# fperezgamonal/flownet2-tf

Hardware: AMD Instinct MI355X
Metric: forward pairs/sec at 512x384 (FlowNet2) (higher is better)
Workload: dtype f16x2 (split fp16 hi+lo operands, 3 fp16 MFMAs per product, fp32 accumulate); 1 GPU; FlowNet2 forward, batch=4 synthetic 512x384 pairs per GPU, seeded synthetic weights; pairs_per_gpu=4, parallelism=dp1 (no collective)

## Files before the change

flownet2-tf_amd/csrc/conv.hip:

```cpp
#include "conv_common.h"
#include <cstdlib>

namespace fn2 {

template <typename T, typename OutT, int TC, int WC, int WP>
__global__ void __launch_bounds__(256) conv_igemm_kernel(const ConvArgs p) {
  constexpr int CH = 16 / (int)sizeof(T);
  constexpr int BC = WC * TC * 16;
  constexpr int BP = WP * 64;
  constexpr int NT = 256;
  static_assert(WC * WP == 4, "4 waves per block");
  constexpr int NPR = BP / 64;
  constexpr int NWR = (BC * 4 + NT - 1) / NT;
  constexpr int WSWZ_BIT = (TC == 4) ? 5 : (TC == 2) ? 4 : 3;
  __shared__ uint4 lds[2][(BC + BP) * 4];

  const int tid = threadIdx.x, lane = tid & 63, wave = tid >> 6;
  const int wc = wave / WP, wp = wave % WP;
  const int cid = tid & 3;

  int pad_y = p.pad, pad_x = p.pad, oy_off = 0, ox_off = 0, osc = 1;
  const T* wgt = reinterpret_cast<const T*>(p.wgt);
  const int phase = blockIdx.z / p.splitk, split = blockIdx.z - phase * p.splitk;
  if (p.deconv) {
// ... 808 lines not shown

}

namespace fn2 {

static bool is_flow_head(const fn2_conv_desc* d) {
  return d->kind == 0 && d->out.c == 2 && d->kh == 3 && d->kw == 3 && d->stride == 1 && d->pad == 1 &&
         d->out.dtype == FN2_F32 && d->act == FN2_ACT_NONE;
}

static bool wants_bp64(const ConvArgs& a, int tile, int phases, int layout) {
  if (layout != 1 || (a.dbg & 32)) return false;
  if (tile < 128) return true;
  const char* e = getenv("FN2_BP64_MIN");
  const int min_blocks = e ? atoi(e) : 96;
  return cdiv(a.M, 64) * (long)(a.cout_pad / 128) * phases >= min_blocks;
}

static int build_args(const fn2_conv_desc* d, ConvArgs* out, int* tile_out, int* phases_out) {
  FN2_REQUIRE(d, "conv2d: null descriptor");
  int rc = check_view(&d->in, "conv2d input");
  if (rc) return rc;
  rc = check_view(&d->out, "conv2d output");
  if (rc) return rc;
  FN2_REQUIRE(d->wgt, "conv2d: null weights");
  FN2_REQUIRE((d->kind >= 0 && d->kind <= 3) || d->kind == 5,
              "conv2d: kind must be 0 (conv), 1 (deconv k4 s2 crop 1), 2 (stem row-run conv), 3 (transpose of a stride-2 conv) "
              "or 5 (deconv k4 s2 crop 1, column phases merged)");
  FN2_REQUIRE(d->in.n == d->out.n, "conv2d: batch mismatch");
  FN2_REQUIRE(d->up_src == nullptr || ((d->kind == 1 || d->kind == 5) && d->up_w != nullptr && d->up_c0 >= 0 &&
                                       d->up_c0 + 2 <= d->out.cs && !d->accumulate),
              "conv2d: up_src rides on a kind-1 / kind-5 transposed conv (up_w set, [up_c0, up_c0 + 2) inside the out buffer)");
  FN2_REQUIRE(d->cin_pad % 8 == 0 && d->cin_pad >= d->in.c, "conv2d: cin_pad must be a multiple of 8 >= Cin");
  FN2_REQUIRE(d->in.cs % 8 == 0 && d->in.c0 % 8 == 0, "conv2d: input channel stride/offset must be multiples of 8");
  if (d->kind != 2)
    FN2_REQUIRE(d->in.c0 + d->cin_pad <= d->in.cs, "conv2d: padded input channels exceed the buffer stride");
  const int esz = dtype_size(d->in.dtype);
  const int CH = 16 / esz;
  FN2_REQUIRE(d->kpad > 0 && d->kpad % (4 * CH) == 0, "conv2d: kpad must be a multiple of one k-step");
  fn2_conv_plan plan;
  rc = fn2_conv2d_plan(d->in.dtype, d->cin_pad, d->out.c, &plan);
  if (rc) return rc;
  const bool wfrag = d->wgt_layout == 2;
  if (wfrag)
    FN2_REQUIRE(plan.layout == 1 && plan.cout_tile >= 64 && d->in.dtype == FN2_F16X2 && d->kind != 2,
                "conv2d: wgt_layout 2 (fragment order) is for split-fp16 layers with more than 32 output channels");
  else
    FN2_REQUIRE(d->wgt_layout == plan.layout, "conv2d: wgt_layout %d does not match fn2_conv2d_plan (%d)", d->wgt_layout,
                plan.layout);
  const int tile = plan.cout_tile;
  FN2_REQUIRE(d->cout_pad % tile == 0 && d->cout_pad >= d->out.c, "conv2d: cout_pad must be a multiple of the cout tile");
  FN2_REQUIRE(d->act == FN2_ACT_NONE || d->act == FN2_ACT_LEAKY, "conv2d: bad activation");
  FN2_REQUIRE(d->out.dtype == d->in.dtype || d->out.dtype == FN2_F32 ||
                  (d->in.dtype == FN2_F32 && d->out.dtype == FN2_F16X2),
              "conv2d: output dtype must be the input dtype, fp32, or split-fp16 from an fp32 stem");
  if (d->in.dtype == FN2_F16X2) FN2_REQUIRE(d->in.cs % 8 == 0 && d->in.c0 % 8 == 0, "conv2d: split-fp16 views are group (8) aligned");
  if (d->out.dtype == FN2_F16X2) FN2_REQUIRE(d->out.cs % 8 == 0 && d->out.c0 % 8 == 0, "conv2d: split-fp16 views are group (8) aligned");

  ConvArgs& a = *out;
  a = ConvArgs{};
  a.KH_KW_hint = 0;
  a.wfrag = wfrag ? 1 : 0;
  a.merged = d->kind == 5 ? 1 : 0;
  a.in = d->in.data; a.wgt = d->wgt; a.bias = d->bias; a.out = d->out.data;
  a.N = d->in.n; a.H = d->in.h; a.W = d->in.w; a.in_cs = d->in.cs; a.in_c0 = d->in.c0;
  a.cin_chunks = d->cin_pad / CH;
  int phases = 1;
  int trim[2] = {0, 0};
  if (d->kind == 0) {
    FN2_REQUIRE(d->kh >= 1 && d->kw >= 1 && d->stride >= 1 && d->pad >= 0, "conv2d: bad kernel geometry");
    a.KH = d->kh; a.KW = d->kw; a.stride = d->stride; a.pad = d->pad;
    a.OH = (d->in.h + 2 * d->pad - d->kh) / d->stride + 1;
    a.OW = (d->in.w + 2 * d->pad - d->kw) / d->stride + 1;
    FN2_REQUIRE(a.OH >= 1 && a.OW >= 1, "conv2d: kernel does not fit");
    FN2_REQUIRE(d->out.h == a.OH && d->out.w == a.OW, "conv2d: output spatial size %dx%d != expected %dx%d",
                d->out.h, d->out.w, a.OH, a.OW);
    a.deconv = 0; a.ph_pad0 = a.ph_pad1 = 0;
  } else if (d->kind == 2) {
    FN2_REQUIRE(d->kh >= 1 && d->kw >= 1 && d->stride >= 1 && d->pad == 0, "stem conv: pad must be baked into the input buffer");
    FN2_REQUIRE(d->in.c0 == 0 && d->in.c == d->in.cs, "stem conv: the input view must be the whole buffer");
    FN2_REQUIRE(d->cin_pad >= d->kw * d->in.cs, "stem conv: run (cin_pad) shorter than kw*cs");
    FN2_REQUIRE(d->wgt_layout == 1, "stem conv: runs on the LDS-DMA kernel only (run must be whole 128-byte lines)");
    a.KH = d->kh; a.KW = 1; a.stride = d->stride; a.pad = 0;
    a.KH_KW_hint = d->kw;
    a.OH = (d->in.h - d->kh) / d->stride + 1;
    a.OW = (d->in.w - d->kw) / d->stride + 1;
    FN2_REQUIRE(a.OH >= 1 && a.OW >= 1, "stem conv: kernel does not fit");
    FN2_REQUIRE(d->out.h == a.OH && d->out.w == a.OW, "stem conv: output spatial size %dx%d != expected %dx%d",
                d->out.h, d->out.w, a.OH, a.OW);
// ... 86 lines not shown
  a.kg = 1;
  if (d->wgt_layout == 1 && tile == 128 && !(a.dbg & 32)) {
    const char* e_kg = getenv("FN2_KG");
    if (!e_kg || atoi(e_kg) != 0) {
      const char* e3 = getenv("FN2_KG3_MAX");
      const char* e2 = getenv("FN2_KG2_MAX");
      const long blocks = (long)cdiv(a.M, 64) * (a.cout_pad / 128) * phases;
      if (blocks <= (e3 ? atoi(e3) : 0)) { a.bp64 = 1; a.kg = 3; }
      else if (blocks <= (e2 ? atoi(e2) : 95)) { a.bp64 = 1; a.kg = 2; }
    }
  }
  if (d->wgt_layout == 1 && tile == 128 && !(a.dbg & 32) && d->in.dtype == FN2_F16X2) {
    const char* e_lo = getenv("FN2_DEEP_MIN");
    const char* e_hi = getenv("FN2_DEEP_MAX");
    const long blocks = (long)cdiv(a.M, 64) * (a.cout_pad / 128) * phases;
    const int lo = e_lo ? atoi(e_lo) : 0, hi = e_hi ? atoi(e_hi) : -1;
    if (blocks >= lo && blocks <= hi) { a.bp64 = 3; a.kg = 1; }
  }
  if (d->wgt_layout == 1 && tile == 128 && a.bp64 == 1 && a.kg == 1) {
    const char* e_ring = getenv("FN2_RING_MAX");
    const int ring_max = e_ring ? atoi(e_ring) : 512;
    const long blocks = (long)cdiv(a.M, 64) * (a.cout_pad / 128) * phases;
    if ((a.dbg & 256) || (blocks >= 384 && blocks <= ring_max)) a.bp64 = 2;
    const char* e_rs = getenv("FN2_RING_SPLIT");
    if (e_rs && blocks >= atoi(e_rs) && blocks < 384) a.bp64 = 2;
  }
  *tile_out = tile;
  *phases_out = phases;
  return FN2_OK;
}

static int preferred_split(const ConvArgs& a, int tile, int phases) {
  if (a.merged) return 1;
  const int bp = tile == 128 ? (a.bp64 ? 64 : 128) : (a.bp64 ? 128 : 256);
  const long blocks = (long)cdiv(a.M, bp) * (a.cout_pad / tile) * phases;
  const char* e_min = getenv("FN2_SPLIT_MINBLOCKS");
  if (blocks >= (e_min ? atoi(e_min) : 384)) return 1;
  if (a.bp64 == 3) {
    const char* e_sl = getenv("FN2_DEEP_SLOTS");
    int s = (int)((e_sl ? atoi(e_sl) : 256) / blocks);
    const int maxs = a.ksteps / 16;
    if (s > maxs) s = maxs;
    if (s > 16) s = 16;
    if (s < 2) return 1;
    const int kper = cdiv(a.ksteps, s);
    return cdiv(a.ksteps, kper);
  }
  if (a.kg > 1) {
    const char* e_nos = getenv("FN2_KG_NOSPLIT");
    if (blocks >= (e_nos ? atoi(e_nos) : 96)) return 1;
    const char* e_sl = getenv("FN2_KG_SLOTS");
    int s = (int)((e_sl ? atoi(e_sl) : 256) / blocks);
    const int maxs = a.ksteps / (12 * a.kg);
    if (s > maxs) s = maxs;
    if (s > 16) s = 16;
    if (s < 2) return 1;
    const int kper = cdiv(a.ksteps, s);
    return cdiv(a.ksteps, kper);
  }
  const char* e = getenv("FN2_SPLIT_SLOTS");
  const char* e_rsl = getenv("FN2_RING_SPLIT_SLOTS");
  const int slots = (tile == 128 && a.bp64 == 2) ? (e_rsl ? atoi(e_rsl) : 512) : e ? atoi(e) : 640;
  int s = (int)(slots / blocks);
  const int maxs = a.ksteps / 8;
  if (s > maxs) s = maxs;
  if (s > 16) s = 16;
// ... 349 lines not shown
```

flownet2-tf_amd/csrc/conv2.hip:

```cpp
#include "conv_common.h"

#include <type_traits>
#include <algorithm>
#include <utility>

#ifndef FN2_X2_ORDER
#define FN2_X2_ORDER 0
#endif
#ifndef FN2_CONV_ABLATE
#define FN2_CONV_ABLATE 0
#endif
#ifndef FN2_SETPRIO
#define FN2_SETPRIO 1
#endif

namespace fn2 {

typedef __attribute__((address_space(3))) void* lptr_t;

constexpr unsigned kOobOffset = 0x80000000u;

typedef int v4i_t __attribute__((ext_vector_type(4)));
typedef unsigned u32x4_t __attribute__((ext_vector_type(4)));

// ... 1348 lines not shown
        av[k] = accr[ai[k]];
      }
#pragma unroll
      for (int k = 0; k < 2; ++k) {
        const int it = min(wave + 8 * k, 9);
        const int ky = it >> 1, o = it & 1;
        const int y = r + 2 - ky;
        float sum = tv[k][0];
        sum += tv[k][1];
        sum += tv[k][2];
        sum += tv[k][3];
        sum += tv[k][4];
        const float v = av[k] + sum;
        if (ok[k]) {
          accr[ai[k]] = fin[k] ? 0.f : v;
          const int ox = x0 + x;
          if (fin[k] && ox < W && !(p.h5_ring && (y == 0 || y == H - 1 || ox == 0 || ox == W - 1)))
            pf[(((size_t)n * H + y) * W + ox) * 2 + o] = v + bias_o[o];
        }
      }
    }
  }
  asm volatile("s_waitcnt vmcnt(0)" ::: "memory");
  if (p.h5_wc != nullptr && !(p.dbg & 16)) {
    const long total = (long)p.N * (2 * W + 2 * (H - 2));
    const long per = (total + gridDim.x - 1) / gridDim.x;
    const long m1 = min(total, (long)(b + 1) * per);
    for (long m = (long)b * per + wave; m < m1; m += 8) h5_ring_pixel(p, m);
  }
#endif
}


template <typename OutT, int SPP>
__global__ void __launch_bounds__(256) conv_rowrun_kernel(const ConvArgs p, const int npieces) {
#if defined(__HIP_DEVICE_COMPILE__)
  using T = x2_t;
  constexpr int BC = 64, BP = 128, TCN = 2;
  constexpr int MAXP = SPP == 4 ? 17 : 9;
  __shared__ uint4 ldsA[2][BC * 8];
  __shared__ uint4 ldsB[2][MAXP * 64];
  const int tid = threadIdx.x, lane = tid & 63;
  const int wave = __builtin_amdgcn_readfirstlane(tid >> 6);
  const T* wgt = reinterpret_cast<const T*>(p.wgt);
  const unsigned wrow_bytes = (unsigned)p.ksteps * 128u;
  int bx = blockIdx.x, by = blockIdx.y;
  {
    const int NT = gridDim.x * gridDim.y, L = blockIdx.x + gridDim.x * blockIdx.y;
    const int xcd = L & 7, chunk = NT >> 3, rem = NT & 7;
    const int Lp = xcd * chunk + min(xcd, rem) + (L >> 3);
    bx = Lp / (int)gridDim.y;
    by = Lp - bx * (int)gridDim.y;
  }
  const int m0 = bx * BP, c0 = by * BC;
  const int tn = m0 / (p.OH * p.OW);
  const int trem = m0 - tn * (p.OH * p.OW);
  const int toy = trem / p.OW, tox = trem - toy * p.OW;

  const v4i_t rsrc_w = make_rsrc(wgt, (int)(p.cout_pad * wrow_bytes));
  const v4i_t rsrc_x = make_rsrc(p.in, p.in_bytes);
  const int lrow = lane >> 3, lphys = lane & 7;
  unsigned woff[2];
#pragma unroll
  for (int j = 0; j < 2; ++j) {
    const int row = wave * 16 + j * 8 + lrow;
    woff[j] = (unsigned)(c0 + row) * wrow_bytes + (unsigned)((lphys ^ ((row >> 1) & 7)) * 16);
  }
  const int nslots = ((BP - 1) * p.stride + p.KH_KW_hint) * SPP;
  const int seg0 = (((tn * p.H + toy * p.stride) * p.W + tox * p.stride) * p.in_cs + p.in_c0) * 4;
  constexpr int NBW = (MAXP + 3) / 4;
  unsigned boff[NBW];
#pragma unroll
  for (int j = 0; j < NBW; ++j) {
    const int q = wave + 4 * j;
    const int P = q * 64 + lane;
    const int Ls = P ^ ((P >> 4) & 15);
    boff[j] = (q < npieces && Ls < nslots) ? (unsigned)(seg0 + Ls * 16) : kOobOffset;
  }
  const int nl = p.cin_chunks >> 3;
  const int ngroups = (p.KH_KW_hint * p.in_cs + 7) >> 3;
  auto issue_B = [&](int ky, uint4* lds) {
    const int toff = ky * p.W * p.in_cs * 4;
#pragma unroll
    for (int j = 0; j < NBW; ++j) {
      const int q = wave + 4 * j;
      if (q < npieces) dma16(rsrc_x, &lds[q * 64], boff[j] == kOobOffset ? kOobOffset : boff[j] + (unsigned)toff, 0);
    }
  };
  auto issue_A = [&](int ky, int l, uint4* lds) {
    const int soff = (ky * nl + l) * 128;
#pragma unroll
    for (int j = 0; j < 2; ++j) dma16(rsrc_w, &lds[(wave * 16 + j * 8) * 8], woff[j], soff);
  };

  const int fr = lane & 31, fh = lane >> 5, fsw = (fr >> 1) & 7;
  const int pslot = (wave * 32 + fr) * p.stride * SPP;
  f32x16 acc[TCN];
#pragma unroll
  for (int tc = 0; tc < TCN; ++tc)
#pragma unroll
    for (int q = 0; q < 16; ++q) acc[tc][q] = 0.f;

  issue_B(0, ldsB[0]);
  issue_A(0, 0, ldsA[0]);
  asm volatile("s_waitcnt vmcnt(0)" ::: "memory");
  __syncthreads();
  int abuf = 0;
  for (int ky = 0; ky < p.KH; ++ky) {
    const uint4* lb = ldsB[ky & 1];
    for (int l = 0; l < nl; ++l) {
      if (l + 1 < nl) issue_A(ky, l + 1, ldsA[abuf ^ 1]);
      else if (ky + 1 < p.KH) issue_A(ky + 1, 0, ldsA[abuf ^ 1]);
      if (l == 0 && ky + 1 < p.KH) issue_B(ky + 1, ldsB[(ky + 1) & 1]);
#if FN2_SETPRIO
      __builtin_amdgcn_s_setprio(1);
#endif
      const uint4* A = &ldsA[abuf][fr * 8];
#pragma unroll
      for (int q = 0; q < 2; ++q) {
        if (4 * l + 2 * q >= ngroups) continue;
        const int chh = (4 * q + 2 * fh) ^ fsw, chl = (4 * q + 2 * fh + 1) ^ fsw;
        const int g = 4 * l + 2 * q + fh;
        const int sh = pslot + 2 * g, sl = sh + 1;
        const uint4 bh = lb[sh ^ ((sh >> 4) & 15)], bl = lb[sl ^ ((sl >> 4) & 15)];
#pragma unroll
        for (int tc = 0; tc < TCN; ++tc) {
          const uint4 ah = A[tc * 32 * 8 + chh], al = A[tc * 32 * 8 + chl];
          acc[tc] = mfma_32x32x16<f16_t>(al, bh, acc[tc]);
          acc[tc] = mfma_32x32x16<f16_t>(ah, bl, acc[tc]);
          acc[tc] = mfma_32x32x16<f16_t>(ah, bh, acc[tc]);
        }
      }
#if FN2_SETPRIO
      __builtin_amdgcn_s_setprio(0);
#endif
      asm volatile("s_waitcnt vmcnt(0)" ::: "memory");
      __syncthreads();
      abuf ^= 1;
    }
  }

  OutT* out = reinterpret_cast<OutT*>(p.out);
  const bool vec16 = (p.out_cs % 8 == 0) && (p.out_c0 % 8 == 0);
  const int ox = tox + wave * 32 + fr;
  constexpr int ERS = 36;
  float* const tl = reinterpret_cast<float*>(&ldsB[0][0]) + wave * (32 * ERS);
  static_assert(4 * 32 * ERS * 4 <= (int)sizeof(ldsB), "epilogue tiles fit the segment buffers");
#pragma unroll
  for (int tc = 0; tc < TCN; ++tc) {
    const int cout_base = c0 + tc * 32 + fh * 16;
    OutT* po = out + (((size_t)tn * p.out_H + toy) * p.out_W + ox) * p.out_cs + p.out_c0 + cout_base;
    float v[16];
#pragma unroll
    for (int q = 0; q < 16; ++q) {
      float x = acc[tc][q] * p.out_scale + ((p.bias != nullptr && cout_base + q < p.Cout) ? p.bias[cout_base + q] : 0.f);
      if (p.act == FN2_ACT_LEAKY) x = leaky(x);
      v[q] = x;
    }
    if (sizeof(OutT) == 4 && vec16 && c0 + tc * 32 + 32 <= p.Cout && !(p.dbg & 4194304)) {
      store16<OutT>(reinterpret_cast<OutT*>(tl + fr * ERS + fh * 16), v);
      const int rr = lane >> 3, ch = lane & 7;
      OutT* ob = out + (((size_t)tn * p.out_H + toy) * p.out_W + tox + wave * 32) * p.out_cs + p.out_c0 + c0 + tc * 32 + ch * 4;
#pragma unroll
      for (int i = 0; i < 4; ++i) {
        const int row = i * 8 + rr;
        *reinterpret_cast<uint4*>(ob + (size_t)row * p.out_cs) = *reinterpret_cast<const uint4*>(tl + row * ERS + ch * 4);
      }
    } else if (vec16 && cout_base + 15 < p.Cout) {
      store16<OutT>(po, v);
    } else {
#pragma unroll
      for (int q = 0; q < 16; ++q)
        if (cout_base + q < p.Cout) store_elem<OutT>(po + q, v[q]);
    }
  }
#endif
}

template <typename OutT>
static bool launch_rowrun(const ConvArgs& a, int tile, int phases, hipStream_t s) {
  if ((a.dbg & 65536) || tile != 64 || phases != 1 || a.deconv || a.KW != 1 || a.KH_KW_hint < 1 || a.splitk != 1 || a.accum || a.wfrag)
    return false;
  if (a.OW % 128 != 0 || (a.in_cs != 8 && a.in_cs != 16)) return false;
  const int spp = a.in_cs / 4;
  const int nl = a.cin_chunks >> 3;
  const int max_slot = 127 * a.stride * spp + 2 * (4 * nl - 1) + 1;
  const int npieces = max_slot / 64 + 1;
  if (npieces > (spp == 4 ? 17 : 9)) return false;
  dim3 grid(a.M / 128, a.cout_pad / 64, 1), block(256);
  if (conv_name_sink().buf) {
    snprintf(conv_name_sink().buf, conv_name_sink().cap, "conv_rowrun_kernel<%s, %d>", is_x2<OutT>::value ? "fn2::x2_t" : "float", spp);
    return true;
  }
  if (spp == 4) hipLaunchKernelGGL((conv_rowrun_kernel<OutT, 4>), grid, block, 0, s, a, npieces);
  else hipLaunchKernelGGL((conv_rowrun_kernel<OutT, 2>), grid, block, 0, s, a, npieces);
  return true;
}

template <typename OutT>
static bool launch_stem(const ConvArgs& a, int tile, int phases, hipStream_t s) {
  if ((a.dbg & 8192) || tile != 64 || phases != 1 || a.deconv || a.KW != 1 || a.splitk != 1 || a.accum ||
      a.ksteps < 1 || a.ksteps > 4 || a.cout_pad != 64)
    return false;
  const int ntiles = cdiv(a.M, 128);
  if (ntiles < 512) return false;
  const char* e = getenv("FN2_STEM_BLOCKS");
  const int blocks = std::min(ntiles, e ? atoi(e) : 256);
  if (conv_name_sink().buf) {
    snprintf(conv_name_sink().buf, conv_name_sink().cap, "conv_stem_kernel<%s, %d>",
             is_x2<OutT>::value ? "fn2::x2_t" : "float", a.ksteps);
    return true;
  }
  switch (a.ksteps) {
    case 1: hipLaunchKernelGGL((conv_stem_kernel<OutT, 1>), dim3(blocks), dim3(256), 0, s, a, ntiles); break;
    case 2: hipLaunchKernelGGL((conv_stem_kernel<OutT, 2>), dim3(blocks), dim3(256), 0, s, a, ntiles); break;
    case 3: hipLaunchKernelGGL((conv_stem_kernel<OutT, 3>), dim3(blocks), dim3(256), 0, s, a, ntiles); break;
    default: hipLaunchKernelGGL((conv_stem_kernel<OutT, 4>), dim3(blocks), dim3(256), 0, s, a, ntiles); break;
  }
  return true;
}

template <typename OutT>
static bool launch_halo(const ConvArgs& a, int tile, int phases, hipStream_t s) {
  if (((a.dbg & 2048) && !a.merged) || a.stride != 1 || a.splitk != 1 || a.kg != 1 || !a.bp64 || a.wfrag || (a.KW != 2 && a.KW != 3)) return false;
  if (a.deconv && (a.kh_ph[0] != a.KH || a.kh_ph[1] != a.KH || a.kw_ph[0] != a.KW || a.kw_ph[1] != a.KW)) return false;
  if (tile == 128 && a.bp64 == 2 && !(a.dbg & 4096)) return false;
  if (a.bp64 == 3) return false;
// ... 114 lines not shown
  if (conv_name_sink().buf) FN2_CONV_NAME("head5_strip_kernel<%d>", a.ksteps / 3);
  else if (a.ksteps == 3) hipLaunchKernelGGL((head5_strip_kernel<1>), dim3(blocks), dim3(512), 0, s, a);
  else hipLaunchKernelGGL((head5_strip_kernel<2>), dim3(blocks), dim3(512), 0, s, a);
  return conv_launched("flow_head5_strip");
}

int launch_head5(const ConvArgs& a, int blocks, hipStream_t s) {
  if (conv_name_sink().buf)
    FN2_CONV_NAME("conv_igemm2_kernel<fn2::x2_t, float, 1, 4, 2, 2, 2, 1, false, false, false, true>");
  else
    hipLaunchKernelGGL((conv_igemm2_kernel<x2_t, float, 1, 4, 2, 2, 2, 1, false, false, false, true>), dim3(blocks, 1, 1), dim3(256), 0,
                       s, a);
  return conv_launched("flow_head5");
}

bool conv_fast_ok(int in_dtype, int cin_pad, int cout) {
  const int esz = dtype_size(in_dtype);
  return cout > 2 && (cin_pad * esz) % 128 == 0;
}

int launch_conv_fast(const ConvArgs& a, int in_dtype, int out_dtype, int tile, int phases, hipStream_t s) {
  if (tile != 128 && tile != 64 && tile != 32) return fail(FN2_ERR_UNSUPPORTED, "conv fast path: cout tile %d", tile);
  if (in_dtype == FN2_F32) return launch2<float, float>(a, tile, phases, s);
  if (in_dtype == FN2_BF16) {
    if (out_dtype == FN2_BF16) return launch2<bf16_t, bf16_t>(a, tile, phases, s);
    return launch2<bf16_t, float>(a, tile, phases, s);
  }
  if (in_dtype == FN2_F16) {
    if (out_dtype == FN2_F16) return launch2<f16_t, f16_t>(a, tile, phases, s);
    return launch2<f16_t, float>(a, tile, phases, s);
  }
  if (out_dtype == FN2_F16X2) {
    if (launch_rowrun<x2_t>(a, tile, phases, s)) return conv_launched("conv_rowrun");
    if (launch_stem<x2_t>(a, tile, phases, s)) return conv_launched("conv_stem");
    if (launch_halo<x2_t>(a, tile, phases, s)) return conv_launched("conv_halo");
    if (a.merged) return fail(FN2_ERR_UNSUPPORTED, "conv2d kind 5: needs the halo kernel (input width a multiple of 128, no split-K)");
    return launch2<x2_t, x2_t>(a, tile, phases, s);
  }
  if (launch_halo<float>(a, tile, phases, s)) return conv_launched("conv_halo");
  if (a.merged) return fail(FN2_ERR_UNSUPPORTED, "conv2d kind 5: needs the halo kernel (input width a multiple of 128, no split-K)");
  return launch2<x2_t, float>(a, tile, phases, s);
}

}
```

flownet2-tf_amd/csrc/elem.hip:

```cpp
#include "fn2_common.h"

namespace fn2 {

__device__ __forceinline__ void warp3(const float* __restrict__ img, long nb, int x, int y, float u, float v,
                                      int W, int H, float o[3]) {
  const float x2 = (float)x + u, y2 = (float)y + v;
  o[0] = o[1] = o[2] = 0.f;
  if (!((x2 >= 0.f) && (y2 >= 0.f) && (x2 < (float)W) && (y2 < (float)H))) return;
  const int xL = (int)x2, yT = (int)y2;
  const int xR = min(xL + 1, W - 1), yB = min(yT + 1, H - 1);
  const float al = x2 - (float)xL, be = y2 - (float)yT;
  const float cTL = (1.f - al) * (1.f - be), cTR = al * (1.f - be), cBL = (1.f - al) * be, cBR = al * be;
  const rgb3_t tl = load_rgb(img + (nb + (long)yT * W + xL) * 3), tr = load_rgb(img + (nb + (long)yT * W + xR) * 3);
  const rgb3_t bl = load_rgb(img + (nb + (long)yB * W + xL) * 3), br = load_rgb(img + (nb + (long)yB * W + xR) * 3);
  o[0] = cTL * tl.r + cTR * tr.r + cBL * bl.r + cBR * br.r;
  o[1] = cTL * tl.g + cTR * tr.g + cBL * bl.g + cBR * br.g;
  o[2] = cTL * tl.b + cTR * tr.b + cBL * bl.b + cBR * br.b;
}

struct FlowSrc { const float* p; int ph, pw; float sy, sx, scale; float* keep; };

__device__ __forceinline__ float2 flow_at(const FlowSrc& f, int n, int y, int x, long pix) {
  if (f.ph == 0) return *reinterpret_cast<const float2*>(f.p + pix * 2);
  const float fy = (float)y * f.sy;
  const int y0 = (int)floorf(fy);
  const int y1 = min(y0 + 1, f.ph - 1);
  const float ly = fy - (float)y0;
  const float2* r0 = reinterpret_cast<const float2*>(f.p) + ((long)n * f.ph + y0) * f.pw;
  const float2* r1 = reinterpret_cast<const float2*>(f.p) + ((long)n * f.ph + y1) * f.pw;
  const float fx = (float)x * f.sx;
  const int x0 = (int)floorf(fx);
  const int x1 = min(x0 + 1, f.pw - 1);
  const float lx = fx - (float)x0;
  float2 r = bilerp_c2(r0[x0], r0[x1], r1[x0], r1[x1], lx, ly, f.scale);
  asm volatile("" : "+v"(r.x), "+v"(r.y));
  if (f.keep != nullptr) *reinterpret_cast<float2*>(f.keep + pix * 2) = r;
  return r;
}

template <typename OutT>
__global__ void __launch_bounds__(256) stack_input_kernel(const float* __restrict__ a, const float* __restrict__ b,
                                                          const FlowSrc flow, OutT* __restrict__ out,
                                                          int N, int H, int W, int out_cs, int out_c0, int pad) {
  const long npix = (long)N * H * W;
  for (long pix = (long)blockIdx.x * blockDim.x + threadIdx.x; pix < npix; pix += (long)gridDim.x * blockDim.x) {
    const int x = (int)(pix % W), y = (int)((pix / W) % H);
    const long nb = (pix / W / H) * (long)H * W;
    const float2 f = flow_at(flow, (int)(pix / W / H), y, x, pix);
    float wv[3];
    warp3(b, nb, x, y, f.x, f.y, W, H, wv);
    float v[16];
    float e = 0.f;
    const rgb3_t pa = load_rgb(a + pix * 3), pb = load_rgb(b + pix * 3);
    const float av3[3] = {pa.r, pa.g, pa.b}, bv3[3] = {pb.r, pb.g, pb.b};
#pragma unroll
    for (int c = 0; c < 3; ++c) {
      const float av = av3[c];
      v[c] = av;
      v[3 + c] = bv3[c];
      v[6 + c] = wv[c];
      const float d = av - wv[c];
      e += d * d;
    }
    v[9] = f.x * 0.05f;
    v[10] = f.y * 0.05f;
    v[11] = sqrtf(e);
    v[12] = v[13] = v[14] = v[15] = 0.f;
    const size_t opix = ((size_t)(pix / W / H) * (H + 2 * pad) + y + pad) * (W + 2 * pad) + x + pad;
    store16<OutT>(out + opix * out_cs + out_c0, v);
  }
}

template <typename OutT>
__global__ void __launch_bounds__(256) fusion_input_kernel(const float* __restrict__ a, const float* __restrict__ b,
                                                           const FlowSrc fsd, const FlowSrc fcss, OutT* __restrict__ out,
                                                           int N, int H, int W, int out_cs, int out_c0, int pad) {
  const long npix = (long)N * H * W;
  for (long pix = (long)blockIdx.x * blockDim.x + threadIdx.x; pix < npix; pix += (long)gridDim.x * blockDim.x) {
    const int x = (int)(pix % W), y = (int)((pix / W) % H);
    const long nb = (pix / W / H) * (long)H * W;
    const float2 sd = flow_at(fsd, (int)(pix / W / H), y, x, pix);
    const float2 cs = flow_at(fcss, (int)(pix / W / H), y, x, pix);
    float wsd[3], wcs[3];
    warp3(b, nb, x, y, sd.x, sd.y, W, H, wsd);
    warp3(b, nb, x, y, cs.x, cs.y, W, H, wcs);
    float v[16];
    float esd = 0.f, ecs = 0.f;
    const rgb3_t pa = load_rgb(a + pix * 3);
    const float av3[3] = {pa.r, pa.g, pa.b};
#pragma unroll
    for (int c = 0; c < 3; ++c) {
      const float av = av3[c];
      v[c] = av;
      const float d1 = av - wsd[c], d2 = av - wcs[c];
      esd += d1 * d1;
      ecs += d2 * d2;
    }
    v[3] = sd.x; v[4] = sd.y; v[5] = cs.x; v[6] = cs.y;
    v[7] = sqrtf(sd.x * sd.x + sd.y * sd.y);
    v[8] = sqrtf(cs.x * cs.x + cs.y * cs.y);
    v[9] = sqrtf(esd);
    v[10] = sqrtf(ecs);
    v[11] = v[12] = v[13] = v[14] = v[15] = 0.f;
    const size_t opix = ((size_t)(pix / W / H) * (H + 2 * pad) + y + pad) * (W + 2 * pad) + x + pad;
    store16<OutT>(out + opix * out_cs + out_c0, v);
  }
}

static inline int grid_for(long work_items, int block) {
  long g = (work_items + block - 1) / block;
  if (g > 256L * 16) g = 256L * 16;
  if (g < 1) g = 1;
  return (int)g;
}

static int check_out16(const fn2_tensor* out, int c, const char* what) {
  FN2_REQUIRE(out && out->data, "%s: null output", what);
  FN2_REQUIRE(out->c == c, "%s: output view must have %d channels", what, c);
  FN2_REQUIRE(out->cs % 8 == 0 && out->c0 % 8 == 0 && out->c0 + 16 <= out->cs,
              "%s: output needs a 16-channel, 8-aligned slot", what);
  FN2_REQUIRE(out->dtype >= FN2_F32 && out->dtype <= FN2_F16X2, "%s: bad dtype", what);
  return FN2_OK;
}

}

using namespace fn2;

template <typename OutT>
__global__ void __launch_bounds__(256) pack_interp_u8_kernel(const unsigned char* __restrict__ img,
                                                             const unsigned char* __restrict__ mask,
                                                             const float* __restrict__ sparse,
                                                             const float* __restrict__ lut,
                                                             const unsigned char* __restrict__ flags,
                                                             OutT* __restrict__ out, int n, int h, int w, int pad,
                                                             int out_cs, int c0) {
  __shared__ float t[512];
  t[threadIdx.x] = (float)threadIdx.x;
  t[256 + threadIdx.x] = lut[threadIdx.x];
  __syncthreads();
  const unsigned npix = (unsigned)n * h * w;
  const int hp = h + 2 * pad, wp = w + 2 * pad;
  for (unsigned i = blockIdx.x * blockDim.x + threadIdx.x; i < npix; i += gridDim.x * blockDim.x) {
    const unsigned row = i / (unsigned)w;
    const int x = (int)(i - row * w), nn = (int)(row / (unsigned)h), y = (int)(row - nn * h);
    const unsigned char* p = img + (size_t)i * 3;
    const unsigned r = p[0], g = p[1], b = p[2], m = mask[i];
    const float2 sf = *reinterpret_cast<const float2*>(sparse + (size_t)i * 2);
    const unsigned ti = flags[2 * nn] ? 256u : 0u, tm = flags[2 * nn + 1] ? 256u : 0u;
    float v[8];
    v[0] = t[ti + r];
    v[1] = t[ti + g];
    v[2] = t[ti + b];
    v[3] = sf.x * 0.05f;
    v[4] = sf.y * 0.05f;
// ... 56 lines not shown
  FN2_REQUIRE(((size_t)out->data & 15) == 0, "pack_interp_u8: output must be 16-byte aligned");
  const int h = out->h - 2 * pad, w = out->w - 2 * pad;
  const long npix = (long)out->n * h * w;
  FN2_REQUIRE(npix < (1L << 31), "pack_interp_u8: more than 2^31 pixels");
  const dim3 g(grid_for(npix, 256)), b(256);
  hipStream_t s = (hipStream_t)stream;
  if (out->dtype == FN2_F32)
    hipLaunchKernelGGL(pack_interp_u8_kernel<float>, g, b, 0, s, img, mask, sparse, lut256, flags, (float*)out->data,
                       out->n, h, w, pad, out->cs, out->c0);
  else if (out->dtype == FN2_F16X2)
    hipLaunchKernelGGL(pack_interp_u8_kernel<x2_t>, g, b, 0, s, img, mask, sparse, lut256, flags, (x2_t*)out->data,
                       out->n, h, w, pad, out->cs, out->c0);
  else if (out->dtype == FN2_BF16)
    hipLaunchKernelGGL(pack_interp_u8_kernel<bf16_t>, g, b, 0, s, img, mask, sparse, lut256, flags, (bf16_t*)out->data,
                       out->n, h, w, pad, out->cs, out->c0);
  else
    hipLaunchKernelGGL(pack_interp_u8_kernel<f16_t>, g, b, 0, s, img, mask, sparse, lut256, flags, (f16_t*)out->data,
                       out->n, h, w, pad, out->cs, out->c0);
  FN2_CHECK_LAUNCH("pack_interp_u8");
  return FN2_OK;
}

static FlowSrc flow_src(const float* p, int ph, int pw, float scale, float* keep, int out_h, int out_w) {
  FlowSrc f{p, ph, pw, 0.f, 0.f, scale, keep};
  if (ph > 0) {
    f.sy = out_h > 1 ? (float)(ph - 1) / (float)(out_h - 1) : 0.f;
    f.sx = out_w > 1 ? (float)(pw - 1) / (float)(out_w - 1) : 0.f;
  }
  return f;
}

static int stack_input_launch(const float* a, const float* b, const FlowSrc& f, const fn2_tensor* out, int pad, void* stream) {
  const long npix = (long)out->n * (out->h - 2 * pad) * (out->w - 2 * pad);
  if (out->dtype == FN2_F32)
    hipLaunchKernelGGL(stack_input_kernel<float>, dim3(grid_for(npix, 256)), dim3(256), 0, (hipStream_t)stream, a,
                       b, f, (float*)out->data, out->n, out->h - 2 * pad, out->w - 2 * pad, out->cs, out->c0, pad);
  else if (out->dtype == FN2_F16X2)
    hipLaunchKernelGGL(stack_input_kernel<x2_t>, dim3(grid_for(npix, 256)), dim3(256), 0, (hipStream_t)stream, a,
                       b, f, (x2_t*)out->data, out->n, out->h - 2 * pad, out->w - 2 * pad, out->cs, out->c0, pad);
  else if (out->dtype == FN2_BF16)
    hipLaunchKernelGGL(stack_input_kernel<bf16_t>, dim3(grid_for(npix, 256)), dim3(256), 0, (hipStream_t)stream, a,
                       b, f, (bf16_t*)out->data, out->n, out->h - 2 * pad, out->w - 2 * pad, out->cs, out->c0, pad);
  else
    hipLaunchKernelGGL(stack_input_kernel<f16_t>, dim3(grid_for(npix, 256)), dim3(256), 0, (hipStream_t)stream, a,
                       b, f, (f16_t*)out->data, out->n, out->h - 2 * pad, out->w - 2 * pad, out->cs, out->c0, pad);
  FN2_CHECK_LAUNCH("stack_input");
  return FN2_OK;
}

int fn2_stack_input(const float* a, const float* b, const float* flow, const fn2_tensor* out, int pad, void* stream) {
  FN2_REQUIRE(a && b && flow, "stack_input: null pointer");
  int rc = check_out16(out, 12, "stack_input");
  if (rc) return rc;
  FN2_REQUIRE(pad >= 0 && out->h > 2 * pad && out->w > 2 * pad, "bad border");
  return stack_input_launch(a, b, flow_src(flow, 0, 0, 1.f, nullptr, 0, 0), out, pad, stream);
}

int fn2_stack_input_pf(const float* a, const float* b, const float* pf, int pf_h, int pf_w, float scale, float* flow_out,
                       const fn2_tensor* out, int pad, void* stream) {
  FN2_REQUIRE(a && b && pf && pf_h >= 1 && pf_w >= 1, "stack_input_pf: null pointer / bad size");
  int rc = check_out16(out, 12, "stack_input_pf");
  if (rc) return rc;
  FN2_REQUIRE(pad >= 0 && out->h > 2 * pad && out->w > 2 * pad, "bad border");
  return stack_input_launch(a, b, flow_src(pf, pf_h, pf_w, scale, flow_out, out->h - 2 * pad, out->w - 2 * pad), out, pad, stream);
}

static int fusion_input_launch(const float* a, const float* b, const FlowSrc& fs, const FlowSrc& fc, const fn2_tensor* out,
                               int pad, void* stream) {
  const long npix = (long)out->n * (out->h - 2 * pad) * (out->w - 2 * pad);
  if (out->dtype == FN2_F32)
    hipLaunchKernelGGL(fusion_input_kernel<float>, dim3(grid_for(npix, 256)), dim3(256), 0, (hipStream_t)stream, a,
                       b, fs, fc, (float*)out->data, out->n, out->h - 2 * pad, out->w - 2 * pad, out->cs, out->c0, pad);
  else if (out->dtype == FN2_F16X2)
    hipLaunchKernelGGL(fusion_input_kernel<x2_t>, dim3(grid_for(npix, 256)), dim3(256), 0, (hipStream_t)stream,
                       a, b, fs, fc, (x2_t*)out->data, out->n, out->h - 2 * pad, out->w - 2 * pad, out->cs, out->c0, pad);
  else if (out->dtype == FN2_BF16)
    hipLaunchKernelGGL(fusion_input_kernel<bf16_t>, dim3(grid_for(npix, 256)), dim3(256), 0, (hipStream_t)stream,
                       a, b, fs, fc, (bf16_t*)out->data, out->n, out->h - 2 * pad, out->w - 2 * pad, out->cs, out->c0, pad);
  else
    hipLaunchKernelGGL(fusion_input_kernel<f16_t>, dim3(grid_for(npix, 256)), dim3(256), 0, (hipStream_t)stream,
                       a, b, fs, fc, (f16_t*)out->data, out->n, out->h - 2 * pad, out->w - 2 * pad, out->cs, out->c0, pad);
  FN2_CHECK_LAUNCH("fusion_input");
  return FN2_OK;
}

int fn2_fusion_input(const float* a, const float* b, const float* flow_sd, const float* flow_css,
                     const fn2_tensor* out, int pad, void* stream) {
  FN2_REQUIRE(a && b && flow_sd && flow_css, "fusion_input: null pointer");
  int rc = check_out16(out, 11, "fusion_input");
  if (rc) return rc;
  FN2_REQUIRE(pad >= 0 && out->h > 2 * pad && out->w > 2 * pad, "bad border");
  return fusion_input_launch(a, b, flow_src(flow_sd, 0, 0, 1.f, nullptr, 0, 0), flow_src(flow_css, 0, 0, 1.f, nullptr, 0, 0),
                             out, pad, stream);
}
// ... 15 lines not shown
```

flownet2-tf_amd/src/engine.py:

```python
import ctypes as C
import os
import types

import numpy as np
import torch

from . import _hip, netdefs, weights as W

_DT = {"f32": torch.float32, "bf16": torch.bfloat16, "f16": torch.float16, "f16x2": torch.float32}
_CODE = {"f32": _hip.FN2_F32, "bf16": _hip.FN2_BF16, "f16": _hip.FN2_F16, "f16x2": _hip.FN2_F16X2}


def _round_up(x, m):
    return (x + m - 1) // m * m


class BatchTooLarge(ValueError):

    def __init__(self, name, batch, nbytes, limit):
        self.fit = max(1, int(batch * (limit - 1) // nbytes))
        super().__init__("activation tensor %s of a batch of %d pairs is %d bytes (limit %d): at most %d pairs per engine"
                         % (name, batch, nbytes, limit, self.fit))


# ... 52 lines not shown
                                 (_hip.ptr(src), _hip.ptr(lut), _hip.ptr(dst), cnt)))
                self.branch_of.append(0)
        self.interp_u8_inputs = bool(interp_u8_inputs)
        if self.interp_u8_inputs:
            if model != "FlowNetS_interp":
                raise ValueError("interp_u8_inputs belongs to FlowNetS_interp, not %s" % model)
            self.in_img_u8 = torch.zeros((self.N, self.H, self.W, 3), dtype=torch.uint8, device=self.device)
            self.in_mask_u8 = torch.zeros((self.N, self.H, self.W), dtype=torch.uint8, device=self.device)
            self.in_sparse = torch.zeros((self.N, self.H, self.W, 2), dtype=torch.float32, device=self.device)
            self.in_flags = torch.ones((self.N, 2), dtype=torch.uint8, device=self.device)
            self._lut_255 = torch.from_numpy((np.arange(256, dtype=np.float64) / 255.0).astype(np.float32)).to(self.device)
        self.graph = None
        self.conv_descs = []
        self.layers = []
        self.heads_as_gemm = heads_as_gemm
        self.plain_stems = bool(plain_stems)
        self.fragment_weights = bool(int(os.environ.get("FN2_WREG", "1"))) if fragment_weights is None else bool(fragment_weights)
        self.compose_heads = bool(heads_as_gemm) and dtype == "f16x2" and bool(int(os.environ.get("FN2_COMPOSE", "1")))
        self._head_t = {}
        self._defer_flow = False
        self._own_ws = set()
        self._pending_head = None
        self.outputs = self._build()
        assert self._pending_head is None
        self._check_variables(strict)
        self._alloc_workspace()
        self._resolve_kernel_names()

    def _buf(self, name, n, h, w, c, dtype=None, stem=False):
        line = 64 if self.act_code in (_hip.FN2_BF16, _hip.FN2_F16) else 32
        cs = (_round_up(c, line) if c > 32 else _round_up(c, 8)) if dtype is None else c
        if dtype is None and not stem and line == 32 and 8 < c <= 32:
            cs = 32

        td = self.tdtype if dtype is None else dtype
        nbytes = n * h * w * cs * torch.empty((), dtype=td).element_size()
        if nbytes >= self.MAX_TENSOR_BYTES:
            if self.N <= 1:
                raise ValueError("one %d x %d pair needs a %d-byte tensor (%s): above the %d-byte limit of the kernels"
                                 % (self.H, self.W, nbytes, name, self.MAX_TENSOR_BYTES))
            raise BatchTooLarge(name, self.N, nbytes, self.MAX_TENSOR_BYTES)
        t = torch.zeros((n, h, w, cs), dtype=td, device=self.device)
        assert name not in self.bufs, name
        self.bufs[name] = t
        self.code_of[t.data_ptr()] = self.act_code if dtype is None else _hip.FN2_F32
        return t

    def _code(self, buf):
        base = buf.untyped_storage().data_ptr()
        return self.code_of.get(buf.data_ptr(), self.code_of.get(base, _hip.dtype_code(buf)))

    def _v(self, buf, c=None, c0=0):
        return _hip.view(buf, c, c0, self._code(buf))

    def _w(self, key):
        if key not in self.weights:
            raise KeyError("the weights lack %r, a variable of the reference's %s graph" % (key, self.model))
        self.consumed.add(key)
        return self.weights[key]

    def _bias(self, scope, name, kind, cout):
        key = f"{scope}/{name}/biases"
        if not netdefs.has_bias(self.model, name, kind, self.no_deconv_biases):
            if key in self.weights:
                self.ignored_variables.append(key)
            return None
# ... 495 lines not shown
        return self._final_flow(tag, preds, 20.0)

    def _net_sd(self, scope, tag, x):
        N, H, W_ = self.N, self.H, self.W
        L = {s[0]: s for s in netdefs.flownet_sd_layers()}
        cats = self._alloc_cats(tag, N)
        c0 = self._buf(f"{tag}/conv0", N, H, W_, 64)
        self._conv_stem(scope, L["conv0"], x, (c0, 0, 64))
        c1 = self._buf(f"{tag}/conv1", N, H // 2, W_ // 2, 64)
        self._conv(scope, L["conv1"], (c0, 0, 64), (c1, 0, 64))
        c1_1 = self._buf(f"{tag}/conv1_1", N, H // 2, W_ // 2, 128)
        self._conv(scope, L["conv1_1"], (c1, 0, 64), (c1_1, 0, 128))
        self._conv(scope, L["conv2"], (c1_1, 0, 128), (cats[2], 0, 128))
        c2_1 = self._buf(f"{tag}/conv2_1", N, H // 4, W_ // 4, 128)
        self._conv(scope, L["conv2_1"], (cats[2], 0, 128), (c2_1, 0, 128))
        c3 = self._buf(f"{tag}/conv3", N, H // 8, W_ // 8, 256)
        self._conv(scope, L["conv3"], (c2_1, 0, 128), (c3, 0, 256))
        self._conv(scope, L["conv3_1"], (c3, 0, 256), (cats[3], 0, 256))
        c6_1 = self._encoder_tail(scope, tag, L, cats)
        preds = self._refine(scope, tag, L, c6_1, cats, True)
        return self._final_flow(tag, preds, 0.05)

    def _pair_input(self, tag, pad):
        x = self._buf(f"{tag}/pair", self.N, self.H + 2 * pad, self.W + 2 * pad, 6, stem=True)
        v = self._v(x, 6, 0)
        self.keep.append(v)
        if self.interp_u8_inputs:
            self._op(f"{tag}/pack_interp_u8", self.lib.fn2_pack_interp_u8, _hip.ptr(self.in_img_u8), _hip.ptr(self.in_mask_u8),
                     _hip.ptr(self.in_sparse), _hip.ptr(self._lut_255), _hip.ptr(self.in_flags), C.byref(v), pad)
            return x
        self._op(f"{tag}/pack_pair", self.lib.fn2_pack_pair, _hip.ptr(self.in_a), _hip.ptr(self.in_b), C.byref(v), pad)
        return x

    def _stacked_input(self, tag, preds):
        x = self._buf(f"{tag}/stack", self.N, self.H + 6, self.W + 6, 16, stem=True)
        v = self._v(x, 12, 0)
        self.keep.append(v)
        if "_flow_src" in preds:
            pf2, scale = preds["_flow_src"]
            self._op(f"{tag}/stack_input", self.lib.fn2_stack_input_pf, _hip.ptr(self.in_a), _hip.ptr(self.in_b), _hip.ptr(pf2),
                     pf2.shape[1], pf2.shape[2], C.c_float(scale), _hip.ptr(preds["flow"]), C.byref(v), 3, kernel="stack_input")
        else:
            self._op(f"{tag}/stack_input", self.lib.fn2_stack_input, _hip.ptr(self.in_a), _hip.ptr(self.in_b),
                     _hip.ptr(preds["flow"]), C.byref(v), 3)
        return x

    def _sub(self, build, *args):
        prev, self._defer_flow = self._defer_flow, bool(int(os.environ.get("FN2_FLOW_IN_CONSUMER", "1")))
        try:
            return build(*args)
        finally:
            self._defer_flow = prev

    def _net_cs(self, scope, tag):
        pc = self._sub(self._net_c, scope + "/FlowNetC", tag + "/C")
        return self._net_s(scope + "/FlowNetS", tag + "/S", self._stacked_input(tag + "/S", pc), 12)

    def _net_css(self, scope, tag):
        pcs = self._sub(self._net_cs, scope + "/FlowNetCS", tag + "/CS")
        return self._net_s(scope + "/FlowNetS", tag + "/S", self._stacked_input(tag + "/S", pcs), 12)

    def _net_2(self, scope, tag):
        N, H, W_ = self.N, self.H, self.W
        fork = len(self.ops)
        css = self._sub(self._net_css, scope + "/FlowNetCSS", tag + "/CSS")
        if self._lanes_on and self._lane_mask & 2:
            fork += min(int(os.environ.get("FN2_SD_FORK_OPS", "0")), len(self.ops) - fork)
            self.syncs.append((fork, 1, 0))
# ... 245 lines not shown
```

Before: 1114 pairs/s.

## Store 12-channel stacked stem input densely and add a 3-slot row-run conv path

The stacked FlowNetS input (12 real channels) is now stored with a 12-channel pixel stride instead of being padded to 16. A new dense stack_input kernel writes pixel pairs, and the row-run stem conv gains an SPP=3 instantiation with its own LDS swizzle and slot rounding. The aim is to cut memory traffic and LDS footprint for the stem conv and the stack writes by a quarter. The cost is stricter alignment requirements (even stride and width), no split-K, and a hard failure if the row-run kernel cannot be used.

```diff
diff --git a/flownet2-tf_amd/csrc/conv.hip b/flownet2-tf_amd/csrc/conv.hip
--- a/flownet2-tf_amd/csrc/conv.hip
+++ b/flownet2-tf_amd/csrc/conv.hip
@@ -864,7 +864,15 @@
                                        d->up_c0 + 2 <= d->out.cs && !d->accumulate),
               "conv2d: up_src rides on a kind-1 / kind-5 transposed conv (up_w set, [up_c0, up_c0 + 2) inside the out buffer)");
   FN2_REQUIRE(d->cin_pad % 8 == 0 && d->cin_pad >= d->in.c, "conv2d: cin_pad must be a multiple of 8 >= Cin");
-  FN2_REQUIRE(d->in.cs % 8 == 0 && d->in.c0 % 8 == 0, "conv2d: input channel stride/offset must be multiples of 8");
+  const bool dense12 = d->kind == 2 && d->in.dtype == FN2_F16X2 && d->out.dtype == FN2_F16X2 && d->in.cs == 12 && d->in.c0 == 0;
+  if (dense12) {
+    FN2_REQUIRE(d->stride % 2 == 0, "stem conv on a 12-channel pixel stride: stride %d is odd (odd output pixels would start mid-group)",
+                d->stride);
+    FN2_REQUIRE(d->in.w % 2 == 0 && reinterpret_cast<size_t>(d->in.data) % 32 == 0,
+                "stem conv on a 12-channel pixel stride: row pitch %d x 48 bytes / base not a multiple of 32 bytes (rows would start mid-group)",
+                d->in.w);
+  }
+  FN2_REQUIRE(dense12 || (d->in.cs % 8 == 0 && d->in.c0 % 8 == 0), "conv2d: input channel stride/offset must be multiples of 8");
   if (d->kind != 2)
     FN2_REQUIRE(d->in.c0 + d->cin_pad <= d->in.cs, "conv2d: padded input channels exceed the buffer stride");
   const int esz = dtype_size(d->in.dtype);
@@ -886,7 +894,7 @@
   FN2_REQUIRE(d->out.dtype == d->in.dtype || d->out.dtype == FN2_F32 ||
                   (d->in.dtype == FN2_F32 && d->out.dtype == FN2_F16X2),
               "conv2d: output dtype must be the input dtype, fp32, or split-fp16 from an fp32 stem");
-  if (d->in.dtype == FN2_F16X2) FN2_REQUIRE(d->in.cs % 8 == 0 && d->in.c0 % 8 == 0, "conv2d: split-fp16 views are group (8) aligned");
+  if (d->in.dtype == FN2_F16X2) FN2_REQUIRE(dense12 || (d->in.cs % 8 == 0 && d->in.c0 % 8 == 0), "conv2d: split-fp16 views are group (8) aligned");
   if (d->out.dtype == FN2_F16X2) FN2_REQUIRE(d->out.cs % 8 == 0 && d->out.c0 % 8 == 0, "conv2d: split-fp16 views are group (8) aligned");
 
   ConvArgs& a = *out;
@@ -1039,6 +1047,7 @@
 
 static int preferred_split(const ConvArgs& a, int tile, int phases) {
   if (a.merged) return 1;
+  if (a.in_cs % 8 != 0) return 1;
   const int bp = tile == 128 ? (a.bp64 ? 64 : 128) : (a.bp64 ? 128 : 256);
   const long blocks = (long)cdiv(a.M, bp) * (a.cout_pad / tile) * phases;
   const char* e_min = getenv("FN2_SPLIT_MINBLOCKS");
diff --git a/flownet2-tf_amd/csrc/conv2.hip b/flownet2-tf_amd/csrc/conv2.hip
--- a/flownet2-tf_amd/csrc/conv2.hip
+++ b/flownet2-tf_amd/csrc/conv2.hip
@@ -1404,12 +1404,18 @@
 }
 
 
+template <int SPP>
+__device__ __forceinline__ int rowrun_swz(int s) {
+  if constexpr (SPP == 3) return s ^ (int)(((unsigned)s / 48u) & 1u);
+  else return s ^ ((s >> 4) & 15);
+}
+
 template <typename OutT, int SPP>
 __global__ void __launch_bounds__(256) conv_rowrun_kernel(const ConvArgs p, const int npieces) {
 #if defined(__HIP_DEVICE_COMPILE__)
   using T = x2_t;
   constexpr int BC = 64, BP = 128, TCN = 2;
-  constexpr int MAXP = SPP == 4 ? 17 : 9;
+  constexpr int MAXP = SPP == 4 ? 17 : SPP == 3 ? 13 : 9;
   __shared__ uint4 ldsA[2][BC * 8];
   __shared__ uint4 ldsB[2][MAXP * 64];
   const int tid = threadIdx.x, lane = tid & 63;
@@ -1438,7 +1444,7 @@
     const int row = wave * 16 + j * 8 + lrow;
     woff[j] = (unsigned)(c0 + row) * wrow_bytes + (unsigned)((lphys ^ ((row >> 1) & 7)) * 16);
   }
-  const int nslots = ((BP - 1) * p.stride + p.KH_KW_hint) * SPP;
+  const int nslots = (((BP - 1) * p.stride + p.KH_KW_hint) * SPP + 1) & ~1;
   const int seg0 = (((tn * p.H + toy * p.stride) * p.W + tox * p.stride) * p.in_cs + p.in_c0) * 4;
   constexpr int NBW = (MAXP + 3) / 4;
   unsigned boff[NBW];
@@ -1446,7 +1452,7 @@
   for (int j = 0; j < NBW; ++j) {
     const int q = wave + 4 * j;
     const int P = q * 64 + lane;
-    const int Ls = P ^ ((P >> 4) & 15);
+    const int Ls = rowrun_swz<SPP>(P);
     boff[j] = (q < npieces && Ls < nslots) ? (unsigned)(seg0 + Ls * 16) : kOobOffset;
   }
   const int nl = p.cin_chunks >> 3;
@@ -1494,7 +1500,7 @@
         const int chh = (4 * q + 2 * fh) ^ fsw, chl = (4 * q + 2 * fh + 1) ^ fsw;
         const int g = 4 * l + 2 * q + fh;
         const int sh = pslot + 2 * g, sl = sh + 1;
-        const uint4 bh = lb[sh ^ ((sh >> 4) & 15)], bl = lb[sl ^ ((sl >> 4) & 15)];
+        const uint4 bh = lb[rowrun_swz<SPP>(sh)], bl = lb[rowrun_swz<SPP>(sl)];
 #pragma unroll
         for (int tc = 0; tc < TCN; ++tc) {
           const uint4 ah = A[tc * 32 * 8 + chh], al = A[tc * 32 * 8 + chl];
@@ -1553,18 +1559,20 @@
 static bool launch_rowrun(const ConvArgs& a, int tile, int phases, hipStream_t s) {
   if ((a.dbg & 65536) || tile != 64 || phases != 1 || a.deconv || a.KW != 1 || a.KH_KW_hint < 1 || a.splitk != 1 || a.accum || a.wfrag)
     return false;
-  if (a.OW % 128 != 0 || (a.in_cs != 8 && a.in_cs != 16)) return false;
+  if (a.OW % 128 != 0 || (a.in_cs != 8 && a.in_cs != 12 && a.in_cs != 16)) return false;
+  if (a.in_cs == 12 && (a.stride % 2 != 0 || a.W % 2 != 0)) return false;
   const int spp = a.in_cs / 4;
   const int nl = a.cin_chunks >> 3;
   const int max_slot = 127 * a.stride * spp + 2 * (4 * nl - 1) + 1;
   const int npieces = max_slot / 64 + 1;
-  if (npieces > (spp == 4 ? 17 : 9)) return false;
+  if (npieces > (spp == 4 ? 17 : spp == 3 ? 13 : 9)) return false;
   dim3 grid(a.M / 128, a.cout_pad / 64, 1), block(256);
   if (conv_name_sink().buf) {
     snprintf(conv_name_sink().buf, conv_name_sink().cap, "conv_rowrun_kernel<%s, %d>", is_x2<OutT>::value ? "fn2::x2_t" : "float", spp);
     return true;
   }
   if (spp == 4) hipLaunchKernelGGL((conv_rowrun_kernel<OutT, 4>), grid, block, 0, s, a, npieces);
+  else if (spp == 3) hipLaunchKernelGGL((conv_rowrun_kernel<OutT, 3>), grid, block, 0, s, a, npieces);
   else hipLaunchKernelGGL((conv_rowrun_kernel<OutT, 2>), grid, block, 0, s, a, npieces);
   return true;
 }
@@ -1745,6 +1753,9 @@
   }
   if (out_dtype == FN2_F16X2) {
     if (launch_rowrun<x2_t>(a, tile, phases, s)) return conv_launched("conv_rowrun");
+    if (a.in_cs % 8 != 0)
+      return fail(FN2_ERR_UNSUPPORTED, "stem conv on a 12-channel pixel stride: needs the row-run kernel (output width a multiple "
+                                       "of 128, 7 x 12 channels in at most three lines)");
     if (launch_stem<x2_t>(a, tile, phases, s)) return conv_launched("conv_stem");
     if (launch_halo<x2_t>(a, tile, phases, s)) return conv_launched("conv_halo");
     if (a.merged) return fail(FN2_ERR_UNSUPPORTED, "conv2d kind 5: needs the halo kernel (input width a multiple of 128, no split-K)");
diff --git a/flownet2-tf_amd/csrc/elem.hip b/flownet2-tf_amd/csrc/elem.hip
--- a/flownet2-tf_amd/csrc/elem.hip
+++ b/flownet2-tf_amd/csrc/elem.hip
@@ -38,6 +38,32 @@
   return r;
 }
 
+__device__ __forceinline__ void stack_pixel(const float* __restrict__ a, const float* __restrict__ b, const FlowSrc& flow,
+                                            long pix, int H, int W, float* v) {
+  const int x = (int)(pix % W), y = (int)((pix / W) % H);
+  const long nb = (pix / W / H) * (long)H * W;
+  const float2 f = flow_at(flow, (int)(pix / W / H), y, x, pix);
+  float wv[3];
+  warp3(b, nb, x, y, f.x, f.y, W, H, wv);
+  float e = 0.f;
+  const rgb3_t pa = load_rgb(a + pix * 3), pb = load_rgb(b + pix * 3);
+  const float av3[3] = {pa.r, pa.g, pa.b}, bv3[3] = {pb.r, pb.g, pb.b};
+#pragma unroll
+  for (int c = 0; c < 3; ++c) {
+    const float av = av3[c];
+    v[c] = av;
+    v[3 + c] = bv3[c];
+    v[6 + c] = wv[c];
+    const float d = av - wv[c];
+    e += d * d;
+  }
+  v[9] = f.x * 0.05f;
+  v[10] = f.y * 0.05f;
+  v[11] = sqrtf(e);
+#pragma unroll
+  for (int c = 0; c < 12; ++c) asm volatile("" : "+v"(v[c]));
+}
+
 template <typename OutT>
 __global__ void __launch_bounds__(256) stack_input_kernel(const float* __restrict__ a, const float* __restrict__ b,
                                                           const FlowSrc flow, OutT* __restrict__ out,
@@ -45,29 +71,38 @@
   const long npix = (long)N * H * W;
   for (long pix = (long)blockIdx.x * blockDim.x + threadIdx.x; pix < npix; pix += (long)gridDim.x * blockDim.x) {
     const int x = (int)(pix % W), y = (int)((pix / W) % H);
-    const long nb = (pix / W / H) * (long)H * W;
-    const float2 f = flow_at(flow, (int)(pix / W / H), y, x, pix);
-    float wv[3];
-    warp3(b, nb, x, y, f.x, f.y, W, H, wv);
     float v[16];
-    float e = 0.f;
-    const rgb3_t pa = load_rgb(a + pix * 3), pb = load_rgb(b + pix * 3);
-    const float av3[3] = {pa.r, pa.g, pa.b}, bv3[3] = {pb.r, pb.g, pb.b};
-#pragma unroll
-    for (int c = 0; c < 3; ++c) {
-      const float av = av3[c];
-      v[c] = av;
-      v[3 + c] = bv3[c];
-      v[6 + c] = wv[c];
-      const float d = av - wv[c];
-      e += d * d;
-    }
-    v[9] = f.x * 0.05f;
-    v[10] = f.y * 0.05f;
-    v[11] = sqrtf(e);
+    stack_pixel(a, b, flow, pix, H, W, v);
     v[12] = v[13] = v[14] = v[15] = 0.f;
     const size_t opix = ((size_t)(pix / W / H) * (H + 2 * pad) + y + pad) * (W + 2 * pad) + x + pad;
     store16<OutT>(out + opix * out_cs + out_c0, v);
+  }
+}
+
+__global__ void __launch_bounds__(256) stack_input_dense_kernel(const float* __restrict__ a, const float* __restrict__ b,
+                                                                const FlowSrc flow, x2_t* __restrict__ out,
+                                                                int N, int H, int W, int pad) {
+  const int j0 = pad >> 1, npair = ((pad + W - 1) >> 1) - j0 + 1;
+  const long total = (long)N * H * npair;
+  for (long i = (long)blockIdx.x * blockDim.x + threadIdx.x; i < total; i += (long)gridDim.x * blockDim.x) {
+    const int j = j0 + (int)(i % npair), y = (int)((i / npair) % H);
+    const long n = i / npair / H;
+    float v[24];
+#pragma unroll
+    for (int k = 0; k < 2; ++k) {
+      const int x = 2 * j + k - pad;
+      if (x >= 0 && x < W) {
+        stack_pixel(a, b, flow, (n * H + y) * W + x, H, W, v + 12 * k);
+      } else {
+#pragma unroll
+        for (int c = 0; c < 12; ++c) v[12 * k + c] = 0.f;
+      }
+    }
+    const size_t opix = ((size_t)n * (H + 2 * pad) + y + pad) * (W + 2 * pad) + 2 * j;
+    uint4* q = reinterpret_cast<uint4*>(out + opix * 12);
+    split8(v, q[0], q[1]);
+    split8(v + 8, q[2], q[3]);
+    split8(v + 16, q[4], q[5]);
   }
 }
 
@@ -121,6 +156,18 @@
               "%s: output needs a 16-channel, 8-aligned slot", what);
   FN2_REQUIRE(out->dtype >= FN2_F32 && out->dtype <= FN2_F16X2, "%s: bad dtype", what);
   return FN2_OK;
+}
+
+static int check_out_stack(const fn2_tensor* out, const char* what) {
+  if (out && out->cs == 12) {
+    FN2_REQUIRE(out->data && out->c == 12, "%s: output view must have 12 channels", what);
+    FN2_REQUIRE(out->dtype == FN2_F16X2, "%s: a 12-channel pixel stride is a split-fp16 layout only", what);
+    FN2_REQUIRE(out->c0 == 0, "%s: a 12-channel pixel stride takes the whole buffer (c0 = 0)", what);
+    FN2_REQUIRE(out->w % 2 == 0 && reinterpret_cast<size_t>(out->data) % 32 == 0,
+                "%s: on a 12-channel pixel stride rows and images must start on 32-byte boundaries (even padded width)", what);
+    return FN2_OK;
+  }
+  return check_out16(out, 12, what);
 }
 
 }
@@ -243,7 +290,11 @@
 
 static int stack_input_launch(const float* a, const float* b, const FlowSrc& f, const fn2_tensor* out, int pad, void* stream) {
   const long npix = (long)out->n * (out->h - 2 * pad) * (out->w - 2 * pad);
-  if (out->dtype == FN2_F32)
+  if (out->cs == 12) {
+    const long npair = (long)out->n * (out->h - 2 * pad) * (((pad + out->w - 2 * pad - 1) >> 1) - (pad >> 1) + 1);
+    hipLaunchKernelGGL(stack_input_dense_kernel, dim3(grid_for(npair, 256)), dim3(256), 0, (hipStream_t)stream, a, b, f,
+                       (x2_t*)out->data, out->n, out->h - 2 * pad, out->w - 2 * pad, pad);
+  } else if (out->dtype == FN2_F32)
     hipLaunchKernelGGL(stack_input_kernel<float>, dim3(grid_for(npix, 256)), dim3(256), 0, (hipStream_t)stream, a,
                        b, f, (float*)out->data, out->n, out->h - 2 * pad, out->w - 2 * pad, out->cs, out->c0, pad);
   else if (out->dtype == FN2_F16X2)
@@ -261,7 +312,7 @@
 
 int fn2_stack_input(const float* a, const float* b, const float* flow, const fn2_tensor* out, int pad, void* stream) {
   FN2_REQUIRE(a && b && flow, "stack_input: null pointer");
-  int rc = check_out16(out, 12, "stack_input");
+  int rc = check_out_stack(out, "stack_input");
   if (rc) return rc;
   FN2_REQUIRE(pad >= 0 && out->h > 2 * pad && out->w > 2 * pad, "bad border");
   return stack_input_launch(a, b, flow_src(flow, 0, 0, 1.f, nullptr, 0, 0), out, pad, stream);
@@ -270,7 +321,7 @@
 int fn2_stack_input_pf(const float* a, const float* b, const float* pf, int pf_h, int pf_w, float scale, float* flow_out,
                        const fn2_tensor* out, int pad, void* stream) {
   FN2_REQUIRE(a && b && pf && pf_h >= 1 && pf_w >= 1, "stack_input_pf: null pointer / bad size");
-  int rc = check_out16(out, 12, "stack_input_pf");
+  int rc = check_out_stack(out, "stack_input_pf");
   if (rc) return rc;
   FN2_REQUIRE(pad >= 0 && out->h > 2 * pad && out->w > 2 * pad, "bad border");
   return stack_input_launch(a, b, flow_src(pf, pf_h, pf_w, scale, flow_out, out->h - 2 * pad, out->w - 2 * pad), out, pad, stream);
diff --git a/flownet2-tf_amd/src/engine.py b/flownet2-tf_amd/src/engine.py
--- a/flownet2-tf_amd/src/engine.py
+++ b/flownet2-tf_amd/src/engine.py
@@ -108,6 +108,8 @@
         cs = (_round_up(c, line) if c > 32 else _round_up(c, 8)) if dtype is None else c
         if dtype is None and not stem and line == 32 and 8 < c <= 32:
             cs = 32
+        if dtype is None and stem and c == 12:
+            cs = 12
 
         td = self.tdtype if dtype is None else dtype
         nbytes = n * h * w * cs * torch.empty((), dtype=td).element_size()
@@ -669,8 +671,25 @@
         self._op(f"{tag}/pack_pair", self.lib.fn2_pack_pair, _hip.ptr(self.in_a), _hip.ptr(self.in_b), C.byref(v), pad)
         return x
 
+    def _dense_stack(self):
+        if self.dtype_name != "f16x2" or self.plain_stems or not int(os.environ.get("FN2_STACK_DENSE", "1")):
+            return False
+        d = _hip.Fn2ConvDesc()
+        plan = _hip.conv_plan(self.act_code, 96, 64)
+        oh, ow = self.H // 2, self.W // 2
+        if (self.H + 6 - 7) // 2 + 1 != oh or (self.W + 6 - 7) // 2 + 1 != ow or plan.layout != 1:
+            return False
+        d.inp = _hip.Fn2Tensor(4096, self.act_code, self.N, self.H + 6, self.W + 6, 12, 12, 0)
+        d.out = _hip.Fn2Tensor(4096, self.act_code, self.N, oh, ow, 64, 64, 0)
+        d.wgt = 4096
+        d.kind, d.kh, d.kw, d.stride, d.pad, d.act = 2, 7, 7, 2, 0, _hip.ACT_LEAKY
+        d.cin_pad, d.cout_pad, d.kpad, d.wgt_layout, d.out_scale = 96, _round_up(64, plan.cout_tile), 7 * 96, 1, 1.0
+        buf = C.create_string_buffer(256)
+        rc = self.lib.fn2_conv2d_kernel_name(C.byref(d), buf, 256)
+        return rc == 0 and buf.value.decode().startswith("conv_rowrun_kernel") and buf.value.decode().endswith(", 3>")
+
     def _stacked_input(self, tag, preds):
-        x = self._buf(f"{tag}/stack", self.N, self.H + 6, self.W + 6, 16, stem=True)
+        x = self._buf(f"{tag}/stack", self.N, self.H + 6, self.W + 6, 12 if self._dense_stack() else 16, stem=True)
         v = self._v(x, 12, 0)
         self.keep.append(v)
         if "_flow_src" in preds:
```

New measurement: 1117 pairs/s (median of 6 runs). About the same (+0.3%).
